# RaulAstudillo06/BOCF

Measured on AMD Instinct MI355X. Metric: acquisition evals/sec (candidates x MC-samples/sec), uEI_noiseless batch call; GP-fit ms alongside, higher is better.
Workload: dtype f64; 1 GPU; BASELINE configs[2]: m=4 rbf-ARD GP, N=4096 d=8, S=1024 MC samples, C=65536 candidates, noise 1e-06, top-16 selection; N=4096, d=8, m=4, S=1024, C=65536, rccl_ranks_seen=0

## Files before the change

### bocf_amd/csrc/gemm_f64.hip

```cpp
#include "bocf_internal.h"

typedef double v4d __attribute__((ext_vector_type(4)));
typedef double v2d __attribute__((ext_vector_type(2)));

#define BM 128
#define BM2 256
#define BN 128
#define BK 16
#define LDT 144
#define QCH 16

template <int EPI, int PF, int NW = 4>
__global__ __launch_bounds__(64 * NW, 2) void gemm_tn_f64_kernel(GemmArgs g) {
  constexpr int JB = NW == 4 ? 4 : 2;
  constexpr int SP = 16 / NW;
  __shared__ double lds[2][2][BK][LDT];

  const int nct = g.Ncols / BN;
  const int nrt = g.M / BM;
  int b = blockIdx.x;
  int rt, ct, batch;
#ifdef BOCF_PROBES
  if (g.swizzle >= 100) {
    const int RT = g.swizzle - 100;
    const int per_z = nrt * nct;
    batch = b / per_z;
    const int bb = b - batch * per_z;
    const int grp = bb / (nct * RT);
    const int t = bb - grp * (nct * RT);
    const int ct_hi = t / (8 * RT);
    const int ri = (t >> 3) % RT;
    ct = ct_hi * 8 + (t & 7);
    rt = grp * RT + ri;
  } else if (g.swizzle == 1) {
    const int nrg = (nrt + 7) >> 3, ncg = (nct + 7) >> 3;
    const int xcd = b & 7, q = b >> 3;
    const int sidx = (q >> 6) * 8 + xcd;
    if (sidx >= nrg * ncg * g.batch) return;
    const int w = q & 63;
    const int cg = sidx % ncg, t = sidx / ncg;
    batch = t % g.batch;
    rt = (t / g.batch) * 8 + (w & 7);
    ct = cg * 8 + (w >> 3);
    if (rt >= nrt || ct >= nct) return;
  } else
#endif
  if (g.swizzle == 2) {
    const int per = nct * g.batch;
    rt = b / per;
    const int rem = b - rt * per;
    batch = rem / nct;
    ct = rem - batch * nct;
  } else if constexpr (EPI == 3) {
    const int per = nct * (nct + 1) / 2;
    batch = b / per;
    int ut = b - batch * per;
    rt = 0;
    while (ut >= nct - rt) {
      ut -= nct - rt;
      ++rt;
    }
    ct = rt + ut;
  } else {
    rt = b / nct;
    ct = b - rt * nct;
    batch = blockIdx.z;
  }
  if (g.rt_desc) rt = nrt - 1 - rt;
  if (g.ct_desc) ct = nct - 1 - ct;
  if (g.upper_only && ct < rt) return;
  int kend = g.kb + g.krt * rt + g.kct * ct;
  if (kend > g.K) kend = g.K;
  const int kbeg = g.kbeg_rt * rt + g.kbeg_ct * ct;
  long offA = (long)batch * g.strideA, offB = (long)batch * g.strideB, offC = (long)batch * g.strideC;
  if (g.batch1 > 0) {
    const int z1 = batch % g.batch1, z2 = batch / g.batch1;
    offA = (long)z1 * g.strideA + (long)z2 * g.strideA2;
    offB = (long)z1 * g.strideB + (long)z2 * g.strideB2;
    offC = (long)z1 * g.strideC + (long)z2 * g.strideC2;
  }

  const double* __restrict__ A = g.A + offA + (long)rt * BM;
  const double* B = g.B + offB + (long)ct * BN;

  const int tid = threadIdx.x;
  const int lane = tid & 63;
  const int wave = tid >> 6;
  const int wr = NW == 4 ? wave >> 1 : wave >> 2, wc = NW == 4 ? wave & 1 : wave & 3;
  const int l15 = lane & 15, lq = lane >> 4;

  const int srow = tid >> 6;
  const int scol = (tid & 63) * 2;

  v4d acc[4][JB];
#pragma unroll
  for (int i = 0; i < 4; ++i)
#pragma unroll
    for (int j = 0; j < JB; ++j) acc[i][j] = (v4d){0.0, 0.0, 0.0, 0.0};

  v2d ra0[SP], rb0[SP], ra1[SP], rb1[SP];
  const unsigned aoff = (unsigned)(((long)srow * g.lda + scol) * 8), boff = (unsigned)(((long)srow * g.ldb + scol) * 8);
  const int lda32 = (int)(g.lda * 8 * NW), ldb32 = (int)(g.ldb * 8 * NW);
  auto gload = [&](v2d (&ra)[SP], v2d (&rb)[SP], int kt) {
    const __amdgpu_buffer_rsrc_t resA = __builtin_amdgcn_make_buffer_rsrc(const_cast<double*>(A + (long)kt * g.lda), 0, -1, 0x00020000);
    const __amdgpu_buffer_rsrc_t resB = __builtin_amdgcn_make_buffer_rsrc(const_cast<double*>(B + (long)kt * g.ldb), 0, -1, 0x00020000);
#pragma unroll
    for (int i = 0; i < SP; ++i) {
      ra[i] = __builtin_bit_cast(v2d, __builtin_amdgcn_raw_buffer_load_b128(resA, aoff, i * lda32, 0));
      rb[i] = __builtin_bit_cast(v2d, __builtin_amdgcn_raw_buffer_load_b128(resB, boff, i * ldb32, 0));
    }
  };
  auto lstore = [&](const v2d (&ra)[SP], const v2d (&rb)[SP], int buf) {
#pragma unroll
    for (int i = 0; i < SP; ++i) {
      *reinterpret_cast<v2d*>(&lds[buf][0][srow + NW * i][scol]) = ra[i];
      *reinterpret_cast<v2d*>(&lds[buf][1][srow + NW * i][scol]) = rb[i];
    }
  };
  auto compute = [&](int cur) {
#pragma unroll
    for (int ks = 0; ks < 4; ++ks) {
      const int kq = ks * 4 + lq;
      double fa[4], fb[JB];
#pragma unroll
      for (int i = 0; i < 4; ++i) fa[i] = lds[cur][0][kq][wr * 64 + i * 16 + l15];
#pragma unroll
      for (int j = 0; j < JB; ++j) fb[j] = lds[cur][1][kq][wc * (16 * JB) + j * 16 + l15];
#pragma unroll
      for (int i = 0; i < 4; ++i)
#pragma unroll
        for (int j = 0; j < JB; ++j)
          acc[i][j] = __builtin_amdgcn_mfma_f64_16x16x4f64(fa[i], fb[j], acc[i][j], 0, 0, 0);
    }
  };

  if constexpr (PF == 2) {
    if (kend > kbeg) {
      gload(ra0, rb0, kbeg);
      if (kbeg + BK < kend) gload(ra1, rb1, kbeg + BK);
      lstore(ra0, rb0, 0);
    }
    __syncthreads();
    for (int kt = kbeg; kt < kend; kt += 2 * BK) {
      if (kt + 2 * BK < kend) gload(ra0, rb0, kt + 2 * BK);
      compute(0);
      if (kt + BK < kend) lstore(ra1, rb1, 1);
      __syncthreads();
      if (kt + BK >= kend) break;
      if (kt + 3 * BK < kend) gload(ra1, rb1, kt + 3 * BK);
      compute(1);
      if (kt + 2 * BK < kend) lstore(ra0, rb0, 0);
      __syncthreads();
    }
  } else {
    if (kend > kbeg) {
      gload(ra0, rb0, kbeg);
      lstore(ra0, rb0, 0);
    }
    __syncthreads();
    int cur = 0;
    for (int kt = kbeg; kt < kend; kt += BK) {
      const bool more = (kt + BK) < kend;
      if (more) gload(ra0, rb0, kt + BK);
      compute(cur);
      if (more) lstore(ra0, rb0, cur ^ 1);
      __syncthreads();
      cur ^= 1;
    }
  }

  if (EPI == 0 || EPI == 3) {
    const double* Cin = g.Cin ? g.Cin + offC : nullptr;
    double* Cout = g.Cout + offC;
    const double alpha = g.alpha, beta = g.beta;
    double* stage = &lds[0][0][0][0];
    __syncthreads();
#pragma unroll
    for (int half = 0; half < 2; ++half) {
      if (wr == half) {
#pragma unroll
        for (int i = 0; i < 4; ++i)
#pragma unroll
          for (int j = 0; j < JB; ++j)
#pragma unroll
            for (int r = 0; r < 4; ++r) stage[(i * 16 + lq + 4 * r) * BN + wc * (16 * JB) + j * 16 + l15] = acc[i][j][r];
      }
      __syncthreads();
      const long row0 = (long)rt * BM + half * 64;
      const long col = (long)ct * BN + lane * 2;
      constexpr int RW = 64 / NW, QC = RW < QCH ? RW : QCH;
#pragma unroll
      for (int q0 = 0; q0 < RW; q0 += QC) {
        v2d cin[QC];
        if (Cin) {
#pragma unroll
          for (int q = 0; q < QC; ++q) cin[q] = *reinterpret_cast<const v2d*>(Cin + (row0 + wave + NW * (q0 + q)) * g.ldc + col);
        }
#pragma unroll
        for (int q = 0; q < QC; ++q) {
          const int rr = wave + NW * (q0 + q);
          v2d v = *reinterpret_cast<const v2d*>(&stage[rr * BN + lane * 2]);
          v[0] = alpha * v[0];
          v[1] = alpha * v[1];
          if (Cin) {
            v[0] += beta * cin[q][0];
            v[1] += beta * cin[q][1];
          }
          *reinterpret_cast<v2d*>(Cout + (row0 + rr) * g.ldc + col) = v;
        }
      }
      __syncthreads();
    }
  } else {
    __syncthreads();
    double* red = &lds[0][0][0][0];
#pragma unroll
    for (int j = 0; j < JB; ++j) {
      double s = 0.0;
#pragma unroll
      for (int i = 0; i < 4; ++i)
#pragma unroll
        for (int r = 0; r < 4; ++r) s = __builtin_fma(acc[i][j][r], acc[i][j][r], s);
      s += __shfl_xor(s, 16, 64);
      s += __shfl_xor(s, 32, 64);
      if (lq == 0) red[wr * 128 + wc * (16 * JB) + j * 16 + l15] = s;
    }
    __syncthreads();
    if (tid < 128) {
      double* out = g.sumsq + (long)batch * g.strideSumsq + (long)rt * g.Ncols + (long)ct * BN;
      out[tid] = red[tid] + red[128 + tid];
    }
  }
}


#ifdef BOCF_PROBES
#define LDA2 272
template <int VPROBE, int PA = 2, int PB = 2>
__global__ __launch_bounds__(512, 1) void gemm_tn_f64_sumsq256_kernel(GemmArgs g) {
  __shared__ double ldsA[2][BK][LDA2];
  __shared__ double ldsB[2][BK][LDT];
  const int nct = g.Ncols / BN;
  const int nrt2 = g.M / BM2;
  const int b = blockIdx.x;
  int rt2 = b / nct;
  const int ct = b - rt2 * nct;
  const int batch = blockIdx.z;
  if (g.rt_desc) rt2 = nrt2 - 1 - rt2;
  const int rtA = 2 * rt2, rtB = 2 * rt2 + 1;
  int kendA = g.kb + g.krt * rtA + g.kct * ct, kendB = g.kb + g.krt * rtB + g.kct * ct;
  if (kendA > g.K) kendA = g.K;
  if (kendB > g.K) kendB = g.K;
  const int kend = kendA > kendB ? kendA : kendB;
  const long offA = (long)batch * g.strideA, offB = (long)batch * g.strideB;
  const double* __restrict__ A = g.A + offA + (long)rt2 * BM2;
  const double* __restrict__ B = g.B + offB + (long)ct * BN;
  const int tid = threadIdx.x;
  const int lane = tid & 63;
  const int wave = tid >> 6;
  const int wr = wave >> 1, wc = wave & 1;
  const int l15 = lane & 15, lq = lane >> 4;
  const int my_kend = wr < 2 ? kendA : kendB;
  const int arow = tid >> 7, acol = (tid & 127) * 2;
  const int brow = tid >> 6, bcol = (tid & 63) * 2;

  v4d acc[4][4];
#pragma unroll
  for (int i = 0; i < 4; ++i)
#pragma unroll
    for (int j = 0; j < 4; ++j) acc[i][j] = (v4d){0.0, 0.0, 0.0, 0.0};
  v2d ra0[4], rb0[2], ra1[4], rb1[2];
  auto gload = [&](v2d (&ra)[4], v2d (&rb)[2], int kt) {
#pragma unroll
    for (int i = 0; i < 4; ++i) ra[i] = *reinterpret_cast<const v2d*>(A + (long)(kt + arow + 4 * i) * g.lda + acol);
#pragma unroll
    for (int i = 0; i < 2; ++i) rb[i] = *reinterpret_cast<const v2d*>(B + (long)(kt + brow + 8 * i) * g.ldb + bcol);
  };
  auto lstore = [&](const v2d (&ra)[4], const v2d (&rb)[2], int buf) {
#pragma unroll
    for (int i = 0; i < 4; ++i) *reinterpret_cast<v2d*>(&ldsA[buf][arow + 4 * i][acol]) = ra[i];
#pragma unroll
    for (int i = 0; i < 2; ++i) *reinterpret_cast<v2d*>(&ldsB[buf][brow + 8 * i][bcol]) = rb[i];
  };
  auto compute = [&](int cur, int ks0, int ks1) {
#pragma unroll
    for (int ks = 0; ks < 4; ++ks) {
      if (ks < ks0 || ks >= ks1) continue;
      const int kq = ks * 4 + lq;
      double fa[4], fb[4];
#pragma unroll
      for (int i = 0; i < 4; ++i) {
        if (VPROBE == 3) {
          fa[i] = 1.0 + kq * 1e-9;
          fb[i] = 2.0 + i;
        } else {
          fa[i] = ldsA[cur][kq][wr * 64 + i * 16 + l15];
          fb[i] = ldsB[cur][kq][wc * 64 + i * 16 + l15];
        }
      }
#pragma unroll
      for (int i = 0; i < 4; ++i)
#pragma unroll
        for (int j = 0; j < 4; ++j) acc[i][j] = __builtin_amdgcn_mfma_f64_16x16x4f64(fa[i], fb[j], acc[i][j], 0, 0, 0);
    }
  };
  double pc[8], pacc = 0.0;
  if (VPROBE == 1) {
#pragma unroll
    for (int q = 0; q < 8; ++q) pc[q] = B[(long)q * g.ldb + bcol] * 1e-3;
  }
  auto valu_probe = [&](int kt) {
    if (VPROBE == 1) {
      const double* __restrict__ xs = g.A + offA + (long)(kt + (wave & 3) * 4) * 8;
#pragma unroll 1
      for (int e = 0; e < 4; ++e) {
        double r2 = 0.0;
#pragma unroll
        for (int q = 0; q < 8; ++q) {
          const double df = xs[e * 8 + q] - pc[q];
          r2 += df * df;
        }
        pacc += exp(-0.5 * r2);
      }
    }
  };
  if (kend > 0) {
    gload(ra0, rb0, 0);
    if (BK < kend) gload(ra1, rb1, BK);
    lstore(ra0, rb0, 0);
  }
  __syncthreads();
  for (int kt = 0; kt < kend; kt += 2 * BK) {
    if (VPROBE != 4 && kt + 2 * BK < kend) gload(ra0, rb0, kt + 2 * BK);
    valu_probe(kt);
    const int pos = wave >= 4 ? PB : PA;
    const bool on0 = kt < my_kend;
    if (pos == 0 && kt + BK < kend) lstore(ra1, rb1, 1);
    if (on0) compute(0, 0, 2);
    if (pos == 1 && kt + BK < kend) lstore(ra1, rb1, 1);
    if (on0) compute(0, 2, 4);
    if (pos == 2 && kt + BK < kend) lstore(ra1, rb1, 1);
    if (VPROBE != 2) __syncthreads();
    if (kt + BK >= kend) break;
    if (VPROBE != 4 && kt + 3 * BK < kend) gload(ra1, rb1, kt + 3 * BK);
    valu_probe(kt + BK);
    const bool on1 = kt + BK < my_kend;
    if (pos == 0 && kt + 2 * BK < kend) lstore(ra0, rb0, 0);
    if (on1) compute(1, 0, 2);
    if (pos == 1 && kt + 2 * BK < kend) lstore(ra0, rb0, 0);
    if (on1) compute(1, 2, 4);
    if (pos == 2 && kt + 2 * BK < kend) lstore(ra0, rb0, 0);
    if (VPROBE != 2) __syncthreads();
  }
  if (VPROBE && pacc == 1.2345e300) g.sumsq[0] = pacc;
  __syncthreads();
  double* red = &ldsA[0][0][0];
#pragma unroll
  for (int j = 0; j < 4; ++j) {
    double sq = 0.0;
#pragma unroll
    for (int i = 0; i < 4; ++i)
#pragma unroll
      for (int r = 0; r < 4; ++r) sq = __builtin_fma(acc[i][j][r], acc[i][j][r], sq);
    sq += __shfl_xor(sq, 16, 64);
    sq += __shfl_xor(sq, 32, 64);
    if (lq == 0) red[wr * 128 + wc * 64 + j * 16 + l15] = sq;
  }
  __syncthreads();
  if (tid < 256) {
    const int half = tid >> 7, col = tid & 127;
    double* out = g.sumsq + (long)batch * g.strideSumsq + (long)(rtA + half) * g.Ncols + (long)ct * BN;
    out[col] = red[(2 * half) * 128 + col] + red[(2 * half + 1) * 128 + col];
  }
}

#endif

template <int V>
struct IC {
  static constexpr int value = V;
};

#define LDA3 256
#define LDT3 128
template <int STORE, int QUEUE = 0>
__global__ __launch_bounds__(512, 1) void gemm_tn_f64_sumsq256x3_kernel(GemmArgs g) {
  static_assert(!(STORE && QUEUE), "the tile queue exists for the sum-of-squares epilogue only");
  __shared__ __attribute__((aligned(16))) double ldsA[3 * BK * LDA3];
  __shared__ __attribute__((aligned(16))) double ldsB[3 * BK * LDT3];
  __shared__ int next_tile;
  const int nct = g.Ncols / BN;
  const int nrt2 = g.M / BM2;
  int b = blockIdx.x;
  v2d ra0[4], rb0[2], ra1[4], rb1[2];
  bool primed = false;
  auto tile_of = [&](int t, int& rt2_, int& ct_, int& batch_) {
    const int per = nrt2 * nct;
    batch_ = t / per;
    const int rem = t - batch_ * per;
    rt2_ = rem / nct;
    ct_ = rem - rt2_ * nct;
  };
 for (;;) {
  int rt2, ct, batch;
  if (QUEUE) {
    tile_of(b, rt2, ct, batch);
  } else if (STORE) {
    const int per = nct * g.batch;
    rt2 = b / per;
    const int rem = b - rt2 * per;
    batch = rem / nct;
    ct = rem - batch * nct;
  } else {
    rt2 = b / nct;
    ct = b - rt2 * nct;
    batch = blockIdx.z;
  }
  if (g.rt_desc) rt2 = nrt2 - 1 - rt2;
  const int rtA = 2 * rt2;
  const int kend = BM2 * (rt2 + 1);
  const int k0 = kend - BM2;
  long offA = (long)batch * g.strideA, offB = (long)batch * g.strideB, offC = (long)batch * g.strideC;
  if (g.batch1 > 0) {
    const int z1 = batch % g.batch1, z2 = batch / g.batch1;
    offA = (long)z1 * g.strideA + (long)z2 * g.strideA2;
    offB = (long)z1 * g.strideB + (long)z2 * g.strideB2;
    offC = (long)z1 * g.strideC + (long)z2 * g.strideC2;
  }
  const double* A = g.A + offA + (long)rt2 * BM2;
  const double* B = g.B + offB + (long)ct * BN;
  const int tid = threadIdx.x;
  const int lane = tid & 63;
  const int wave = __builtin_amdgcn_readfirstlane(tid >> 6);
  const int wr = wave >> 1, wc = wave & 1;
  const int l15 = lane & 15, lq = lane >> 4;
  const int sl = tid & 15;
  const int arow = tid >> 7, swr = (tid >> 4) & 3, sh = (tid >> 6) & 1;
  const int brow = tid >> 6, sp = (tid >> 4) & 1, bw = (tid >> 5) & 1;
  const int stA = arow * LDA3 + sh * 128 + swr * 32 + sl * 2, stB = brow * LDT3 + bw * 64 + sp * 32 + sl * 2;
  const int fgA = lq * LDA3 + wr * 32 + l15 * 2, fgB = lq * LDT3 + wc * 64 + l15 * 2;
  int stA2h = (stA >> 1) + BK * LDA3, fgA2h = (fgA >> 1) + BK * LDA3;
  asm volatile("" : "+v"(stA2h), "+v"(fgA2h));
  const int stA2 = stA2h * 2, fgA2 = fgA2h * 2;

  v4d acc[4][4];
#pragma unroll
  for (int i = 0; i < 4; ++i)
#pragma unroll
    for (int j = 0; j < 4; ++j) acc[i][j] = (v4d){0.0, 0.0, 0.0, 0.0};
  const unsigned aoff = (unsigned)(((long)arow * g.lda + sh * 128 + swr * 16 + sl) * 8);
  const unsigned boff = (unsigned)(((long)brow * g.ldb + bw * 64 + sp * 32 + sl) * 8);
  const int lda8 = g.lda * 8, ldb8 = g.ldb * 8;
  auto fetch = [&](v2d (&ra)[4], v2d (&rb)[2], const double* pa, const double* pb) {
    const __amdgpu_buffer_rsrc_t resA = __builtin_amdgcn_make_buffer_rsrc(const_cast<double*>(pa), 0, -1, 0x00020000);
    const __amdgpu_buffer_rsrc_t resB = __builtin_amdgcn_make_buffer_rsrc(const_cast<double*>(pb), 0, -1, 0x00020000);
#pragma unroll
    for (int i = 0; i < 4; ++i) {
      ra[i][0] = __builtin_bit_cast(double, __builtin_amdgcn_raw_buffer_load_b64(resA, aoff, 4 * i * lda8, 0));
      ra[i][1] = __builtin_bit_cast(double, __builtin_amdgcn_raw_buffer_load_b64(resA, aoff + 512u, 4 * i * lda8, 0));
    }
#pragma unroll
    for (int i = 0; i < 2; ++i) {
      rb[i][0] = __builtin_bit_cast(double, __builtin_amdgcn_raw_buffer_load_b64(resB, boff, 8 * i * ldb8, 0));
      rb[i][1] = __builtin_bit_cast(double, __builtin_amdgcn_raw_buffer_load_b64(resB, boff + 128u, 8 * i * ldb8, 0));
    }
  };
  auto frag = [&](double (&a)[4], double (&bb)[4], auto bufc, auto ksc) {
    constexpr int BUF = decltype(bufc)::value, ROW = BUF * BK + decltype(ksc)::value * 4;
    const double* pa = BUF == 2 ? &ldsA[(ROW - 2 * BK) * LDA3 + fgA2] : &ldsA[ROW * LDA3 + fgA];
    const v2d a01 = *reinterpret_cast<const v2d*>(pa), a23 = *reinterpret_cast<const v2d*>(pa + 128);
    const v2d b01 = *reinterpret_cast<const v2d*>(&ldsB[ROW * LDT3 + fgB]), b23 = *reinterpret_cast<const v2d*>(&ldsB[ROW * LDT3 + fgB + 32]);
    a[0] = a01[0], a[1] = a01[1], a[2] = a23[0], a[3] = a23[1];
    bb[0] = b01[0], bb[1] = b01[1], bb[2] = b23[0], bb[3] = b23[1];
  };
  double xa[4], xb[4], ya[4], yb[4];
  auto interleave = [&](auto nmc) {
    constexpr int NM = decltype(nmc)::value;
#pragma unroll
    for (int ks = 0; ks < 4; ++ks) {
      const int nmem = ks < 3 ? 10 : 4;
      const int per = NM >= nmem ? 1 : (nmem + NM - 1) / NM;
      int done = 0;
#pragma unroll
      for (int n = 0; n < NM; ++n) {
        __builtin_amdgcn_sched_group_barrier(0x008, 1, 0);
#pragma unroll
        for (int e = 0; e < per; ++e) {
          if (done < nmem) {
            if (done < 4) __builtin_amdgcn_sched_group_barrier(0x100, 1, 0);
            else if (done == 4 || done == 7) __builtin_amdgcn_sched_group_barrier(0x200, 1, 0);
            else __builtin_amdgcn_sched_group_barrier(0x020, 1, 0);
            ++done;
          }
        }
      }
    }
  };
  const long tileA = (long)BK * g.lda, tileB = (long)BK * g.ldb;
  const double* pA = A + (long)(4 * BK) * g.lda;
  const double* pB = B + (long)(4 * BK) * g.ldb;
  auto step = [&](v2d (&ra)[4], v2d (&rb)[2], int kt, auto curc) {
    constexpr int CUR = decltype(curc)::value, NX = (CUR + 1) % 3, NN = (CUR + 2) % 3;
    const __amdgpu_buffer_rsrc_t resA = __builtin_amdgcn_make_buffer_rsrc(const_cast<double*>(pA), 0, -1, 0x00020000);
    const __amdgpu_buffer_rsrc_t resB = __builtin_amdgcn_make_buffer_rsrc(const_cast<double*>(pB), 0, -1, 0x00020000);
    pA += tileA;
    pB += tileB;
    auto mma = [&](const double (&a)[4], const double (&bb)[4]) {
#pragma unroll
      for (int i = 0; i < 4; ++i)
#pragma unroll
        for (int j = 0; j < 4; ++j) acc[i][j] = __builtin_amdgcn_mfma_f64_16x16x4f64(a[i], bb[j], acc[i][j], 0, 0, 0);
    };
    auto stA_ = [&](int i) {
      if (NN == 2) *reinterpret_cast<v2d*>(&ldsA[4 * i * LDA3 + stA2]) = ra[i];
      else *reinterpret_cast<v2d*>(&ldsA[(NN * BK + 4 * i) * LDA3 + stA]) = ra[i];
    };
    auto ldA_ = [&](int i) {
      ra[i][0] = __builtin_bit_cast(double, __builtin_amdgcn_raw_buffer_load_b64(resA, aoff, 4 * i * lda8, 0));
      ra[i][1] = __builtin_bit_cast(double, __builtin_amdgcn_raw_buffer_load_b64(resA, aoff + 512u, 4 * i * lda8, 0));
    };
    auto stB_ = [&](int i) {
      *reinterpret_cast<v2d*>(&ldsB[(NN * BK + 8 * i) * LDT3 + stB]) = rb[i];
    };
    auto ldB_ = [&](int i) {
      rb[i][0] = __builtin_bit_cast(double, __builtin_amdgcn_raw_buffer_load_b64(resB, boff, 8 * i * ldb8, 0));
      rb[i][1] = __builtin_bit_cast(double, __builtin_amdgcn_raw_buffer_load_b64(resB, boff + 128u, 8 * i * ldb8, 0));
    };
    frag(ya, yb, IC<CUR>(), IC<1>());
    mma(xa, xb);
    stA_(0), ldA_(0), stA_(1), ldA_(1);
    frag(xa, xb, IC<CUR>(), IC<2>());
    mma(ya, yb);
    stA_(2), ldA_(2), stA_(3), ldA_(3);
    frag(ya, yb, IC<CUR>(), IC<3>());
    mma(xa, xb);
    stB_(0), ldB_(0), stB_(1), ldB_(1);
    frag(xa, xb, IC<NX>(), IC<0>());
    mma(ya, yb);
    interleave(IC<16>());
    __builtin_amdgcn_sched_barrier(0);
    __syncthreads();
  };
  auto dstep = [&](v2d (&ra)[4], v2d (&rb)[2], int kt, int cur) {
    const int tau = (kt - k0) / BK;
    const int qmin = (tau - wr + 3) >> 2;
    const int nx = cur == 2 ? 0 : cur + 1, nn = nx == 2 ? 0 : nx + 1;
    const __amdgpu_buffer_rsrc_t resA = __builtin_amdgcn_make_buffer_rsrc(const_cast<double*>(pA), 0, -1, 0x00020000);
    const __amdgpu_buffer_rsrc_t resB = __builtin_amdgcn_make_buffer_rsrc(const_cast<double*>(pB), 0, -1, 0x00020000);
    const bool adv = kt + 5 * BK < kend;
    pA += adv ? tileA : 0;
    pB += adv ? tileB : 0;
    const double* fa_c = &ldsA[cur * (BK * LDA3) + fgA];
    const double* fb_c = &ldsB[cur * (BK * LDT3) + fgB];
    const double* fa_n = &ldsA[nx * (BK * LDA3) + fgA];
    const double* fb_n = &ldsB[nx * (BK * LDT3) + fgB];
    double* sa = &ldsA[nn * (BK * LDA3) + stA];
    double* sb = &ldsB[nn * (BK * LDT3) + stB];
    auto fragp = [&](double (&a)[4], double (&bb)[4], const double* pa, const double* pb, int ks) {
      const v2d a01 = *reinterpret_cast<const v2d*>(pa + ks * 4 * LDA3), a23 = *reinterpret_cast<const v2d*>(pa + ks * 4 * LDA3 + 128);
      const v2d b01 = *reinterpret_cast<const v2d*>(pb + ks * 4 * LDT3), b23 = *reinterpret_cast<const v2d*>(pb + ks * 4 * LDT3 + 32);
      a[0] = a01[0], a[1] = a01[1], a[2] = a23[0], a[3] = a23[1];
      bb[0] = b01[0], bb[1] = b01[1], bb[2] = b23[0], bb[3] = b23[1];
    };
    auto stld = [&](int i) {
      if (i < 4) {
        *reinterpret_cast<v2d*>(sa + 4 * i * LDA3) = ra[i];
        ra[i][0] = __builtin_bit_cast(double, __builtin_amdgcn_raw_buffer_load_b64(resA, aoff, 4 * i * lda8, 0));
        ra[i][1] = __builtin_bit_cast(double, __builtin_amdgcn_raw_buffer_load_b64(resA, aoff + 512u, 4 * i * lda8, 0));
      } else {
        *reinterpret_cast<v2d*>(sb + 8 * (i - 4) * LDT3) = rb[i - 4];
        rb[i - 4][0] = __builtin_bit_cast(double, __builtin_amdgcn_raw_buffer_load_b64(resB, boff, 8 * (i - 4) * ldb8, 0));
        rb[i - 4][1] = __builtin_bit_cast(double, __builtin_amdgcn_raw_buffer_load_b64(resB, boff + 128u, 8 * (i - 4) * ldb8, 0));
      }
    };
    auto k4 = [&](const double (&a)[4], const double (&bb)[4], int ks) {
#pragma unroll
      for (int q = 0; q < 4; ++q) {
        if (q >= qmin) {
#pragma unroll
          for (int j = 0; j < 4; ++j) acc[q][j] = __builtin_amdgcn_mfma_f64_16x16x4f64(a[q], bb[j], acc[q][j], 0, 0, 0);
        }
        if (ks < 3 && q < 2) stld(2 * ks + q);
      }
    };
    fragp(ya, yb, fa_c, fb_c, 1);
    k4(xa, xb, 0);
    fragp(xa, xb, fa_c, fb_c, 2);
    k4(ya, yb, 1);
    fragp(ya, yb, fa_c, fb_c, 3);
    k4(xa, xb, 2);
    fragp(xa, xb, fa_n, fb_n, 0);
    k4(ya, yb, 3);
    __syncthreads();
  };
  if (!(QUEUE && primed)) {
    fetch(ra0, rb0, A, B);
    fetch(ra1, rb1, A + tileA, B + tileB);
  }
#pragma unroll
  for (int i = 0; i < 4; ++i) *reinterpret_cast<v2d*>(&ldsA[4 * i * LDA3 + stA]) = ra0[i];
#pragma unroll
  for (int i = 0; i < 2; ++i) *reinterpret_cast<v2d*>(&ldsB[8 * i * LDT3 + stB]) = rb0[i];
  fetch(ra0, rb0, A + 2 * tileA, B + 2 * tileB);
#pragma unroll
  for (int i = 0; i < 4; ++i) *reinterpret_cast<v2d*>(&ldsA[(BK + 4 * i) * LDA3 + stA]) = ra1[i];
#pragma unroll
  for (int i = 0; i < 2; ++i) *reinterpret_cast<v2d*>(&ldsB[(BK + 8 * i) * LDT3 + stB]) = rb1[i];
  fetch(ra1, rb1, A + 3 * tileA, B + 3 * tileB);
  __syncthreads();
  frag(xa, xb, IC<0>(), IC<0>());
  const int nfull = k0 / BK, rounds = nfull / 6, rest = nfull - 6 * rounds;
  int kt = 0;
  for (int it = 0; it < rounds; ++it, kt += 6 * BK) {
    step(ra0, rb0, kt, IC<0>());
    step(ra1, rb1, kt + BK, IC<1>());
    step(ra0, rb0, kt + 2 * BK, IC<2>());
    step(ra1, rb1, kt + 3 * BK, IC<0>());
    step(ra0, rb0, kt + 4 * BK, IC<1>());
    step(ra1, rb1, kt + 5 * BK, IC<2>());
  }
  if (rest >= 2) {
    step(ra0, rb0, kt, IC<0>());
    step(ra1, rb1, kt + BK, IC<1>());
  }
  if (rest >= 4) {
    step(ra0, rb0, kt + 2 * BK, IC<2>());
    step(ra1, rb1, kt + 3 * BK, IC<0>());
  }
  int claimed = 0;
  if (QUEUE && tid == 0) claimed = (int)gridDim.x + atomicAdd(g.tile_ctr, 1);
  {
    int cur = rest == 0 ? 0 : (rest == 2 ? 2 : 1);
    for (kt = k0; kt < kend; kt += 2 * BK) {
      dstep(ra0, rb0, kt, cur);
      cur = cur == 2 ? 0 : cur + 1;
      dstep(ra1, rb1, kt + BK, cur);
      cur = cur == 2 ? 0 : cur + 1;
    }
  }
  if (STORE) {
    double* stage = ldsA;
    double* Cout = g.Cout + offC + (long)rt2 * BM2 * g.ldc + (long)ct * BN;
    const double alpha = g.alpha;
    __syncthreads();
#pragma unroll
    for (int pass = 0; pass < 4; ++pass) {
#pragma unroll
      for (int j = 0; j < 4; ++j)
#pragma unroll
        for (int r = 0; r < 4; ++r) stage[(16 * wr + 4 * r + lq) * LDT3 + wc * 64 + 16 * j + l15] = acc[pass][j][r];
      __syncthreads();
#pragma unroll
      for (int e = 0; e < 8; ++e) {
        const int rr = wave + 8 * e;
        v2d v = *reinterpret_cast<const v2d*>(&stage[rr * LDT3 + lane * 2]);
        v[0] *= alpha;
        v[1] *= alpha;
        *reinterpret_cast<v2d*>(Cout + (long)(64 * pass + rr) * g.ldc + lane * 2) = v;
      }
      __syncthreads();
    }
    return;
  }
  double* xfer = ldsA;
  double* red = ldsA + 4 * 4 * 2 * 64;
  int nb = 0;
  if (QUEUE && tid == 0) next_tile = claimed;
#pragma unroll 1
  for (int stage = 0; stage < 4; ++stage) {
    if (wr == stage) {
#pragma unroll
      for (int q = 0; q < 4; ++q)
#pragma unroll
        for (int j = 0; j < 4; ++j) {
          double* slot = xfer + ((q * 4 + j) * 2 + wc) * 64 + lane;
          double sq = stage == 0 ? 0.0 : *slot;
#pragma unroll
          for (int r = 0; r < 4; ++r) sq = __builtin_fma(acc[q][j][r], acc[q][j][r], sq);
          if (stage < 3) {
            *slot = sq;
          } else {
            sq += __shfl_xor(sq, 16, 64);
            sq += __shfl_xor(sq, 32, 64);
            if (lq == 0) red[q * 128 + wc * 64 + j * 16 + l15] = sq;
          }
        }
    }
    __syncthreads();
    if (QUEUE && stage == 0) {
      nb = __builtin_amdgcn_readfirstlane(next_tile);
      primed = nb < nrt2 * nct * g.batch;
      if (primed) {
        int nrt, nc, nz;
        tile_of(nb, nrt, nc, nz);
        if (g.rt_desc) nrt = nrt2 - 1 - nrt;
        const double* An = g.A + (long)nz * g.strideA + (long)nrt * BM2;
        const double* Bn = g.B + (long)nz * g.strideB + (long)nc * BN;
        fetch(ra0, rb0, An, Bn);
        fetch(ra1, rb1, An + tileA, Bn + tileB);
      }
    }
  }
  if (tid < 256) {
    const int half = tid >> 7, col = tid & 127;
    double* out = g.sumsq + (long)batch * g.strideSumsq + (long)(rtA + half) * g.Ncols + (long)ct * BN;
    out[col] = red[(2 * half) * 128 + col] + red[(2 * half + 1) * 128 + col];
  }
  if (!QUEUE) return;
  if (!primed) break;
  b = nb;
  __syncthreads();
 }
  if (threadIdx.x == 0 && atomicAdd(g.tile_ctr + 1, 1) == (int)gridDim.x - 1) {
    __hip_atomic_store(g.tile_ctr, 0, __ATOMIC_RELAXED, __HIP_MEMORY_SCOPE_AGENT);
    __hip_atomic_store(g.tile_ctr + 1, 0, __ATOMIC_RELAXED, __HIP_MEMORY_SCOPE_AGENT);
  }
}

void launch_gemm_f64(const GemmArgs& g0, int batch, int epilogue, hipStream_t s) {
  GemmArgs g = g0;
  g.batch = batch;
  const int nrt = g.M / BM, nct = g.Ncols / BN;
  if (nrt == 0 || nct == 0 || batch == 0) return;
  if (g.swizzle >= 256) {
    if (epilogue == 1 && !g.prefetch1 && g.M % BM2 == 0 && g.kbeg_rt == 0 && g.kbeg_ct == 0 && g.batch1 == 0) {
      const dim3 grid256((unsigned)((g.M / BM2) * nct), 1, (unsigned)batch);
#ifdef BOCF_PROBES
#define L256(V, A, B) BOCF_LAUNCH((gemm_tn_f64_sumsq256_kernel<V, A, B>), grid256, dim3(512), 0, s, g)
      if (g.swizzle != 258 || g.vprobe) {
        g.stagger = g.swizzle == 257 ? 1 : 0;
        if (g.vprobe == 1) L256(1, 2, 2);
        else if (g.vprobe == 2) L256(2, 2, 2);
        else if (g.vprobe == 3) L256(3, 2, 2);
        else if (g.vprobe == 4) L256(4, 2, 2);
        else if (g.stagger == 1) L256(0, 2, 0);
        else L256(0, 2, 2);
        return;
      }
#undef L256
#endif
      if (g.kb == BM && g.krt == BM && g.kct == 0 && g.K >= g.M) {
        const long tiles = (long)(g.M / BM2) * nct * batch;
        if (g.tile_ctr && g.ncu > 0 && tiles <= 0x7fffffffL - g.ncu)
          BOCF_LAUNCH((gemm_tn_f64_sumsq256x3_kernel<0, 1>), dim3((unsigned)(tiles < g.ncu ? tiles : g.ncu)), dim3(512), 0, s, g);
        else
          BOCF_LAUNCH((gemm_tn_f64_sumsq256x3_kernel<0>), grid256, dim3(512), 0, s, g);
        return;
      }
    }
    g.swizzle = 0;
  }
  if (epilogue == 0 && !g.no_x3 && !g.Cin && g.M % BM2 == 0 && g.M >= 2 * BM2 && g.kb == BM && g.krt == BM && g.kct == 0 && g.kbeg_rt == 0 && g.kbeg_ct == 0 &&
      g.K >= g.M && !g.upper_only && g.rt_desc && !g.ct_desc) {
    const dim3 grid256((unsigned)((g.M / BM2) * nct * batch), 1, 1);
    BOCF_LAUNCH((gemm_tn_f64_sumsq256x3_kernel<1>), grid256, dim3(512), 0, s, g);
    return;
  }
  if (epilogue == 3) {
    BOCF_LAUNCH((gemm_tn_f64_kernel<3, 1, 8>), dim3((unsigned)(nct * (nct + 1) / 2 * batch)), dim3(512), 0, s, g);
    return;
  }
  dim3 grid((unsigned)(nrt * nct), 1, (unsigned)batch);
#ifdef BOCF_PROBES
  if (g.swizzle >= 100 && (nct % 8 != 0 || nrt % (g.swizzle - 100) != 0)) g.swizzle = 0;
  if (g.swizzle >= 100) {
    grid = dim3((unsigned)(nrt * nct * batch), 1, 1);
  } else if (g.swizzle == 1) {
    const long ns = (long)((nrt + 7) / 8) * ((nct + 7) / 8) * batch;
    grid = dim3((unsigned)(((ns + 7) / 8) * 8 * 64), 1, 1);
  }
#else
  if (g.swizzle != 2) g.swizzle = 0;
#endif
  if (g.swizzle == 2) grid = dim3((unsigned)(nrt * nct * batch), 1, 1);
  if (epilogue == 0)
    BOCF_LAUNCH((gemm_tn_f64_kernel<0, 1, 8>), grid, dim3(512), 0, s, g);
  else if (g.prefetch1)
    BOCF_LAUNCH((gemm_tn_f64_kernel<1, 1>), grid, dim3(256), 0, s, g);
  else
    BOCF_LAUNCH((gemm_tn_f64_kernel<1, 2>), grid, dim3(256), 0, s, g);
}
```

Measured before the change: 1.094 billion evals/s.

## Prefetch next queued tile during final k-steps and streamline sum-of-squares epilogue

In the persistent tile-queue sum-of-squares GEMM kernel, the next tile is now claimed and its first K-slices are loaded inside the last few diagonal k-steps instead of after the epilogue. This hides the next tile's global-load latency behind the current tile's MFMA tail. The epilogue is rewritten as a wavefront-staggered reduction through LDS that writes outputs directly, replacing the separate red buffer and final store pass. Clock64 phase-timing probes are added under a compile-time probe flag. The change adds tricky buffer-reuse and synchronisation logic (the xfer region overlaps the staged prefetch buffers), which risks correctness or register pressure.

```diff
diff --git a/bocf_amd/csrc/gemm_f64.hip b/bocf_amd/csrc/gemm_f64.hip
--- a/bocf_amd/csrc/gemm_f64.hip
+++ b/bocf_amd/csrc/gemm_f64.hip
@@ -1,4 +1,9 @@
 #include "bocf_internal.h"
+#ifdef BOCF_PROBES
+#include <cstdio>
+#include <cstdlib>
+#include <vector>
+#endif
 
 typedef double v4d __attribute__((ext_vector_type(4)));
 typedef double v2d __attribute__((ext_vector_type(2)));
@@ -383,6 +388,17 @@
 
 #define LDA3 256
 #define LDT3 128
+#ifdef BOCF_PROBES
+__device__ long long* g_tile_phases = nullptr;
+#define TILE_STAMP(k)                          \
+  if (QUEUE == 2) {                            \
+    const long long t_ = clock64();            \
+    if ((k) != 3 || ph_n) ph[k] += t_ - ph_t;  \
+    ph_t = t_;                                 \
+  }
+#else
+#define TILE_STAMP(k)
+#endif
 template <int STORE, int QUEUE = 0>
 __global__ __launch_bounds__(512, 1) void gemm_tn_f64_sumsq256x3_kernel(GemmArgs g) {
   static_assert(!(STORE && QUEUE), "the tile queue exists for the sum-of-squares epilogue only");
@@ -394,6 +410,13 @@
   int b = blockIdx.x;
   v2d ra0[4], rb0[2], ra1[4], rb1[2];
   bool primed = false;
+  int nb = 0;
+  bool primed_next = false;
+  const double *nA = nullptr, *nB = nullptr;
+#ifdef BOCF_PROBES
+  long long ph[4] = {0, 0, 0, 0}, ph_t = 0;
+  int ph_n = 0;
+#endif
   auto tile_of = [&](int t, int& rt2_, int& ct_, int& batch_) {
     const int per = nrt2 * nct;
     batch_ = t / per;
@@ -402,6 +425,7 @@
     ct_ = rem - rt2_ * nct;
   };
  for (;;) {
+  TILE_STAMP(3)
   int rt2, ct, batch;
   if (QUEUE) {
     tile_of(b, rt2, ct, batch);
@@ -545,8 +569,10 @@
     const int tau = (kt - k0) / BK;
     const int qmin = (tau - wr + 3) >> 2;
     const int nx = cur == 2 ? 0 : cur + 1, nn = nx == 2 ? 0 : nx + 1;
-    const __amdgpu_buffer_rsrc_t resA = __builtin_amdgcn_make_buffer_rsrc(const_cast<double*>(pA), 0, -1, 0x00020000);
-    const __amdgpu_buffer_rsrc_t resB = __builtin_amdgcn_make_buffer_rsrc(const_cast<double*>(pB), 0, -1, 0x00020000);
+    const bool tail = QUEUE && tau >= 12;
+    const bool do_st = !QUEUE || tau < 14, do_ld = !tail || (tau < 14 && primed_next);
+    const __amdgpu_buffer_rsrc_t resA = __builtin_amdgcn_make_buffer_rsrc(const_cast<double*>(tail ? nA + (tau - 12) * tileA : pA), 0, -1, 0x00020000);
+    const __amdgpu_buffer_rsrc_t resB = __builtin_amdgcn_make_buffer_rsrc(const_cast<double*>(tail ? nB + (tau - 12) * tileB : pB), 0, -1, 0x00020000);
     const bool adv = kt + 5 * BK < kend;
     pA += adv ? tileA : 0;
     pB += adv ? tileB : 0;
@@ -564,13 +590,17 @@
     };
     auto stld = [&](int i) {
       if (i < 4) {
-        *reinterpret_cast<v2d*>(sa + 4 * i * LDA3) = ra[i];
-        ra[i][0] = __builtin_bit_cast(double, __builtin_amdgcn_raw_buffer_load_b64(resA, aoff, 4 * i * lda8, 0));
-        ra[i][1] = __builtin_bit_cast(double, __builtin_amdgcn_raw_buffer_load_b64(resA, aoff + 512u, 4 * i * lda8, 0));
+        if (do_st) *reinterpret_cast<v2d*>(sa + 4 * i * LDA3) = ra[i];
+        if (do_ld) {
+          ra[i][0] = __builtin_bit_cast(double, __builtin_amdgcn_raw_buffer_load_b64(resA, aoff, 4 * i * lda8, 0));
+          ra[i][1] = __builtin_bit_cast(double, __builtin_amdgcn_raw_buffer_load_b64(resA, aoff + 512u, 4 * i * lda8, 0));
+        }
       } else {
-        *reinterpret_cast<v2d*>(sb + 8 * (i - 4) * LDT3) = rb[i - 4];
-        rb[i - 4][0] = __builtin_bit_cast(double, __builtin_amdgcn_raw_buffer_load_b64(resB, boff, 8 * (i - 4) * ldb8, 0));
-        rb[i - 4][1] = __builtin_bit_cast(double, __builtin_amdgcn_raw_buffer_load_b64(resB, boff + 128u, 8 * (i - 4) * ldb8, 0));
+        if (do_st) *reinterpret_cast<v2d*>(sb + 8 * (i - 4) * LDT3) = rb[i - 4];
+        if (do_ld) {
+          rb[i - 4][0] = __builtin_bit_cast(double, __builtin_amdgcn_raw_buffer_load_b64(resB, boff, 8 * (i - 4) * ldb8, 0));
+          rb[i - 4][1] = __builtin_bit_cast(double, __builtin_amdgcn_raw_buffer_load_b64(resB, boff + 128u, 8 * (i - 4) * ldb8, 0));
+        }
       }
     };
     auto k4 = [&](const double (&a)[4], const double (&bb)[4], int ks) {
@@ -596,18 +626,18 @@
   if (!(QUEUE && primed)) {
     fetch(ra0, rb0, A, B);
     fetch(ra1, rb1, A + tileA, B + tileB);
-  }
-#pragma unroll
-  for (int i = 0; i < 4; ++i) *reinterpret_cast<v2d*>(&ldsA[4 * i * LDA3 + stA]) = ra0[i];
-#pragma unroll
-  for (int i = 0; i < 2; ++i) *reinterpret_cast<v2d*>(&ldsB[8 * i * LDT3 + stB]) = rb0[i];
-  fetch(ra0, rb0, A + 2 * tileA, B + 2 * tileB);
-#pragma unroll
-  for (int i = 0; i < 4; ++i) *reinterpret_cast<v2d*>(&ldsA[(BK + 4 * i) * LDA3 + stA]) = ra1[i];
-#pragma unroll
-  for (int i = 0; i < 2; ++i) *reinterpret_cast<v2d*>(&ldsB[(BK + 8 * i) * LDT3 + stB]) = rb1[i];
-  fetch(ra1, rb1, A + 3 * tileA, B + 3 * tileB);
-  __syncthreads();
+#pragma unroll
+    for (int i = 0; i < 4; ++i) *reinterpret_cast<v2d*>(&ldsA[4 * i * LDA3 + stA]) = ra0[i];
+#pragma unroll
+    for (int i = 0; i < 2; ++i) *reinterpret_cast<v2d*>(&ldsB[8 * i * LDT3 + stB]) = rb0[i];
+    fetch(ra0, rb0, A + 2 * tileA, B + 2 * tileB);
+#pragma unroll
+    for (int i = 0; i < 4; ++i) *reinterpret_cast<v2d*>(&ldsA[(BK + 4 * i) * LDA3 + stA]) = ra1[i];
+#pragma unroll
+    for (int i = 0; i < 2; ++i) *reinterpret_cast<v2d*>(&ldsB[(BK + 8 * i) * LDT3 + stB]) = rb1[i];
+    fetch(ra1, rb1, A + 3 * tileA, B + 3 * tileB);
+    __syncthreads();
+  }
   frag(xa, xb, IC<0>(), IC<0>());
   const int nfull = k0 / BK, rounds = nfull / 6, rest = nfull - 6 * rounds;
   int kt = 0;
@@ -627,17 +657,33 @@
     step(ra0, rb0, kt + 2 * BK, IC<2>());
     step(ra1, rb1, kt + 3 * BK, IC<0>());
   }
+  TILE_STAMP(0)
   int claimed = 0;
   if (QUEUE && tid == 0) claimed = (int)gridDim.x + atomicAdd(g.tile_ctr, 1);
   {
     int cur = rest == 0 ? 0 : (rest == 2 ? 2 : 1);
     for (kt = k0; kt < kend; kt += 2 * BK) {
+      if (QUEUE) {
+        if (kt == k0 + 8 * BK && tid == 0) next_tile = claimed;
+        if (kt == k0 + 10 * BK) {
+          nb = __builtin_amdgcn_readfirstlane(next_tile);
+          primed_next = nb < nrt2 * nct * g.batch;
+          if (primed_next) {
+            int nrt, nc, nz;
+            tile_of(nb, nrt, nc, nz);
+            if (g.rt_desc) nrt = nrt2 - 1 - nrt;
+            nA = g.A + (long)nz * g.strideA + (long)nrt * BM2;
+            nB = g.B + (long)nz * g.strideB + (long)nc * BN;
+          }
+        }
+      }
       dstep(ra0, rb0, kt, cur);
       cur = cur == 2 ? 0 : cur + 1;
       dstep(ra1, rb1, kt + BK, cur);
       cur = cur == 2 ? 0 : cur + 1;
     }
   }
+  TILE_STAMP(1)
   if (STORE) {
     double* stage = ldsA;
     double* Cout = g.Cout + offC + (long)rt2 * BM2 * g.ldc + (long)ct * BN;
@@ -662,10 +708,62 @@
     }
     return;
   }
+  if (QUEUE) {
+    double* xfer = ldsA + 2 * BK * LDA3;
+    if (primed_next) {
+#pragma unroll
+      for (int i = 0; i < 4; ++i) *reinterpret_cast<v2d*>(&ldsA[4 * i * LDA3 + stA]) = ra0[i];
+#pragma unroll
+      for (int i = 0; i < 2; ++i) *reinterpret_cast<v2d*>(&ldsB[8 * i * LDT3 + stB]) = rb0[i];
+      fetch(ra0, rb0, nA + 2 * tileA, nB + 2 * tileB);
+#pragma unroll
+      for (int i = 0; i < 4; ++i) *reinterpret_cast<v2d*>(&ldsA[(BK + 4 * i) * LDA3 + stA]) = ra1[i];
+#pragma unroll
+      for (int i = 0; i < 2; ++i) *reinterpret_cast<v2d*>(&ldsB[(BK + 8 * i) * LDT3 + stB]) = rb1[i];
+      fetch(ra1, rb1, nA + 3 * tileA, nB + 3 * tileB);
+    }
+    double* out = g.sumsq + (long)batch * g.strideSumsq + (long)rtA * g.Ncols + (long)ct * BN + wc * 64 + l15;
+    double half0[4];
+#pragma unroll
+    for (int t = 0; t < 7; ++t) {
+#pragma unroll
+      for (int q = 0; q < 4; ++q) {
+        const int i = t - q;
+        if (i < 0 || i > 3) continue;
+        if (wr == i) {
+          double sq[4];
+#pragma unroll
+          for (int j = 0; j < 4; ++j) sq[j] = i == 0 ? 0.0 : xfer[((q * 4 + j) * 2 + wc) * 64 + lane];
+#pragma unroll
+          for (int j = 0; j < 4; ++j)
+#pragma unroll
+            for (int r = 0; r < 4; ++r) sq[j] = __builtin_fma(acc[q][j][r], acc[q][j][r], sq[j]);
+#pragma unroll
+          for (int j = 0; j < 4; ++j) {
+            if (i < 3) {
+              xfer[((q * 4 + j) * 2 + wc) * 64 + lane] = sq[j];
+            } else {
+              sq[j] += __shfl_xor(sq[j], 16, 64);
+              sq[j] += __shfl_xor(sq[j], 32, 64);
+              if (!(q & 1)) half0[j] = sq[j];
+              else if (lq == 0) out[(long)(q >> 1) * g.Ncols + j * 16] = half0[j] + sq[j];
+            }
+          }
+        }
+      }
+      __syncthreads();
+    }
+    TILE_STAMP(2)
+#ifdef BOCF_PROBES
+    ++ph_n;
+#endif
+    if (!primed_next) break;
+    primed = true;
+    b = nb;
+    continue;
+  }
   double* xfer = ldsA;
   double* red = ldsA + 4 * 4 * 2 * 64;
-  int nb = 0;
-  if (QUEUE && tid == 0) next_tile = claimed;
 #pragma unroll 1
   for (int stage = 0; stage < 4; ++stage) {
     if (wr == stage) {
@@ -687,30 +785,21 @@
         }
     }
     __syncthreads();
-    if (QUEUE && stage == 0) {
-      nb = __builtin_amdgcn_readfirstlane(next_tile);
-      primed = nb < nrt2 * nct * g.batch;
-      if (primed) {
-        int nrt, nc, nz;
-        tile_of(nb, nrt, nc, nz);
-        if (g.rt_desc) nrt = nrt2 - 1 - nrt;
-        const double* An = g.A + (long)nz * g.strideA + (long)nrt * BM2;
-        const double* Bn = g.B + (long)nz * g.strideB + (long)nc * BN;
-        fetch(ra0, rb0, An, Bn);
-        fetch(ra1, rb1, An + tileA, Bn + tileB);
-      }
-    }
   }
   if (tid < 256) {
     const int half = tid >> 7, col = tid & 127;
     double* out = g.sumsq + (long)batch * g.strideSumsq + (long)(rtA + half) * g.Ncols + (long)ct * BN;
     out[col] = red[(2 * half) * 128 + col] + red[(2 * half + 1) * 128 + col];
   }
-  if (!QUEUE) return;
-  if (!primed) break;
-  b = nb;
-  __syncthreads();
+  return;
  }
+#ifdef BOCF_PROBES
+  if (QUEUE == 2 && threadIdx.x == 0 && g_tile_phases) {
+    long long* o = g_tile_phases + 5 * (long)blockIdx.x;
+    for (int k = 0; k < 4; ++k) o[k] = ph[k];
+    o[4] = ph_n;
+  }
+#endif
   if (threadIdx.x == 0 && atomicAdd(g.tile_ctr + 1, 1) == (int)gridDim.x - 1) {
     __hip_atomic_store(g.tile_ctr, 0, __ATOMIC_RELAXED, __HIP_MEMORY_SCOPE_AGENT);
     __hip_atomic_store(g.tile_ctr + 1, 0, __ATOMIC_RELAXED, __HIP_MEMORY_SCOPE_AGENT);
@@ -741,10 +830,32 @@
 #endif
       if (g.kb == BM && g.krt == BM && g.kct == 0 && g.K >= g.M) {
         const long tiles = (long)(g.M / BM2) * nct * batch;
-        if (g.tile_ctr && g.ncu > 0 && tiles <= 0x7fffffffL - g.ncu)
+        if (g.tile_ctr && g.ncu > 0 && tiles <= 0x7fffffffL - g.ncu) {
+#ifdef BOCF_PROBES
+          if (const char* path = getenv("BOCF_TILE_PHASES")) {
+            const int nwg = (int)(tiles < g.ncu ? tiles : g.ncu);
+            long long* dev = nullptr;
+            if (hipMalloc((void**)&dev, sizeof(long long) * 5 * nwg) != hipSuccess) return;
+            (void)hipMemsetAsync(dev, 0, sizeof(long long) * 5 * nwg, s);
+            (void)hipMemcpyToSymbol(HIP_SYMBOL(g_tile_phases), &dev, sizeof(dev));
+            BOCF_LAUNCH((gemm_tn_f64_sumsq256x3_kernel<0, 2>), dim3((unsigned)nwg), dim3(512), 0, s, g);
+            std::vector<long long> host(5 * (size_t)nwg);
+            (void)hipStreamSynchronize(s);
+            (void)hipMemcpy(host.data(), dev, sizeof(long long) * 5 * nwg, hipMemcpyDeviceToHost);
+            (void)hipFree(dev);
+            if (FILE* f = fopen(path, "a")) {
+              fprintf(f, "launch M %d Ncols %d batch %d workgroups %d\n", g.M, g.Ncols, batch, nwg);
+              for (int w = 0; w < nwg; ++w)
+                fprintf(f, "%d %lld %lld %lld %lld %lld\n", w, host[5 * w], host[5 * w + 1], host[5 * w + 2], host[5 * w + 3], host[5 * w + 4]);
+              fclose(f);
+            }
+            return;
+          }
+#endif
           BOCF_LAUNCH((gemm_tn_f64_sumsq256x3_kernel<0, 1>), dim3((unsigned)(tiles < g.ncu ? tiles : g.ncu)), dim3(512), 0, s, g);
-        else
+        } else {
           BOCF_LAUNCH((gemm_tn_f64_sumsq256x3_kernel<0>), grid256, dim3(512), 0, s, g);
+        }
         return;
       }
     }
```

Result: slower. 1.082 billion evals/s (-1.1%).
